# KogarashiNetwork/Kogarashi

Hardware: AMD Instinct MI355X
Metric: bn254_g1_msm_pairs_per_sec (higher is better)
Workload: dtype u32x9 (29-bit limbs)

## Files before the change

### kogarashi_amd/csrc/curve.h

```cpp
#pragma once
#include "fp29.h"
#include "fp_inv.h"

namespace kg {

template <class F>
struct Affine {
  F x, y;
};

template <class F>
struct XYZZ {
  F x, y, zz, zzz;
  static KG_HD XYZZ identity() { return {F::zero(), F::zero(), F::zero(), F::zero()}; }
};

template <class F>
KG_HD bool is_identity(const XYZZ<F>& p) { return is_zero_2p(p.zz); }

template <class F>
KG_HD XYZZ<F> from_affine(const Affine<F>& a) { return {a.x, a.y, F::one(), F::one()}; }

template <class F>
KG_HD XYZZ<F> double_affine(const Affine<F>& a) {
// ... 12 lines not shown
KG_HD XYZZ<F> double_xyzz(const XYZZ<F>& p) {
  if (is_identity(p)) return p;
  F u = norm(dbl(p.y));
  F v = sqr(u);
  F w = mul(u, v);
  F s = mul(p.x, v);
  F xx = sqr(p.x);
  F m = norm(add(dbl(xx), xx));
  F x3 = vred(norm(sub<4, 1>(sqr(m), norm(dbl(s)))));
  F y3 = vred(norm(sub<4, 1>(mul(m, norm(sub<4, 1>(s, x3))), mul(w, p.y))));
  return {x3, y3, mul(v, p.zz), mul(w, p.zzz)};
}

template <class F>
KG_HD XYZZ<F> add_mixed(const XYZZ<F>& p, const Affine<F>& a) {
  if (is_identity(p)) return from_affine(a);
  F u2 = mul(a.x, p.zz);
  F s2 = mul(a.y, p.zzz);
  F pp_ = norm(sub<4, 1>(u2, p.x));
  F r = norm(sub<4, 1>(s2, p.y));
  F pp = sqr(pp_);
  if (is_zero_2p(pp)) {
    if (is_zero(r)) return double_affine(a);
    return XYZZ<F>::identity();
  }
  F ppp = mul(pp_, pp);
  F q = mul(p.x, pp);
  F x3 = vred(norm(sub<8, 3>(sqr(r), add(ppp, dbl(q)))));
  F y3 = mul2sub(r, norm(sub<4, 1>(q, x3)), p.y, ppp);
  return {x3, y3, mul(p.zz, pp), mul(p.zzz, ppp)};
}

template <class F>
KG_HD XYZZ<F> add_mixed_signed(const XYZZ<F>& p, const Affine<F>& a, bool negate) {
  if (is_identity(p)) return from_affine(negate ? neg_affine(a) : a);
  F u2 = mul(a.x, p.zz);
  F s2 = mul(a.y, p.zzz);
  F pp_ = norm(sub<8, 1>(u2, p.x));
  F t = negate ? sub<8, 1>(F::zero(), s2) : s2;
  F r = norm(sub<4, 1>(t, p.y));
  F pp = sqr(pp_);
  if (is_zero_2p(pp)) {
    if (is_zero(r)) return double_affine(negate ? neg_affine(a) : a);
    return XYZZ<F>::identity();
  }
  F ppp = mul(pp_, pp);
  F q = mul(p.x, pp);
  F x3 = norm(sub<4, 3>(sqr(r), add(ppp, dbl(q))));
  F y3 = mul2sub(r, norm(sub<8, 1>(q, x3)), p.y, ppp);
  return {x3, y3, mul(p.zz, pp), mul(p.zzz, ppp)};
}

template <class G>
KG_HD XYZZ<Fp2<G>> add_mixed_signed(const XYZZ<Fp2<G>>& p, const Affine<Fp2<G>>& a, bool negate) {
  return add_mixed(p, negate ? neg_affine(a) : a);
}

template <class F>
KG_HD XYZZ<F> add_xyzz(const XYZZ<F>& p, const XYZZ<F>& q_) {
  if (is_identity(p)) return q_;
  if (is_identity(q_)) return p;
  F u1 = mul(p.x, q_.zz);
  F u2 = mul(q_.x, p.zz);
  F s1 = mul(p.y, q_.zzz);
  F s2 = mul(q_.y, p.zzz);
  F pp_ = norm(sub<4, 1>(u2, u1));
  F r = norm(sub<4, 1>(s2, s1));
  F pp = sqr(pp_);
  if (is_zero_2p(pp)) {
    if (is_zero(r)) return double_xyzz(p);
    return XYZZ<F>::identity();
  }
  F ppp = mul(pp_, pp);
  F q = mul(u1, pp);
  F x3 = vred(norm(sub<8, 3>(sqr(r), add(ppp, dbl(q)))));
  F y3 = mul2sub(r, norm(sub<4, 1>(q, x3)), s1, ppp);
  return {x3, y3, mul(mul(p.zz, q_.zz), pp), mul(mul(p.zzz, q_.zzz), ppp)};
}

#if defined(__HIP_DEVICE_COMPILE__)
#define KG_STREAM_FENCE() __asm__ volatile("" ::: "memory")
#else
#define KG_STREAM_FENCE() ((void)0)
#endif
// ... 83 lines not shown
```

### kogarashi_amd/csrc/fp29.h

```cpp
#pragma once
#include <type_traits>
#include <cstdint>
#include "fp_consts.h"

#if defined(__HIPCC__)
#include <hip/hip_runtime.h>
#define KG_HD __host__ __device__ __forceinline__
#else
#define KG_HD inline __attribute__((always_inline))
#endif

namespace kg {

constexpr uint32_t M29 = 0x1fffffffu;

template <class P>
struct Fp {
  using Params = P;
  uint32_t l[9];

  static KG_HD Fp zero() {
    Fp r;
#pragma unroll
    for (int i = 0; i < 9; ++i) r.l[i] = 0;
// ... 367 lines not shown
#pragma unroll
  for (int i = 0; i < 9; ++i) {
    z |= a.l[i];
    e |= a.l[i] ^ P::P[i];
  }
  return z == 0 || e == 0;
}
template <class P>
KG_HD bool is_zero(const Fp<P>& a) { return is_zero_2p(mul(a, Fp<P>::one())); }

template <class P>
KG_HD bool same_limbs(const Fp<P>& a, const Fp<P>& b) {
  uint32_t e = 0;
#pragma unroll
  for (int i = 0; i < 9; ++i) e |= a.l[i] ^ b.l[i];
  return e == 0;
}

template <class P>
KG_HD Fp<P> limbs_from_words(const uint32_t w[8]) {
  Fp<P> r;
  r.l[0] = w[0] & M29;
  r.l[1] = ((w[0] >> 29) | (w[1] << 3)) & M29;
  r.l[2] = ((w[1] >> 26) | (w[2] << 6)) & M29;
  r.l[3] = ((w[2] >> 23) | (w[3] << 9)) & M29;
  r.l[4] = ((w[3] >> 20) | (w[4] << 12)) & M29;
  r.l[5] = ((w[4] >> 17) | (w[5] << 15)) & M29;
  r.l[6] = ((w[5] >> 14) | (w[6] << 18)) & M29;
  r.l[7] = ((w[6] >> 11) | (w[7] << 21)) & M29;
  r.l[8] = w[7] >> 8;
  return r;
}
template <class P>
KG_HD void words_from_limbs(const Fp<P>& a, uint32_t w[8]) {
  w[0] = a.l[0] | (a.l[1] << 29);
  w[1] = (a.l[1] >> 3) | (a.l[2] << 26);
  w[2] = (a.l[2] >> 6) | (a.l[3] << 23);
  w[3] = (a.l[3] >> 9) | (a.l[4] << 20);
  w[4] = (a.l[4] >> 12) | (a.l[5] << 17);
  w[5] = (a.l[5] >> 15) | (a.l[6] << 14);
  w[6] = (a.l[6] >> 18) | (a.l[7] << 11);
  w[7] = (a.l[7] >> 21) | (a.l[8] << 8);
}
template <class P>
KG_HD Fp<P> from_ref(const uint32_t w[8]) { return mul(limbs_from_words<P>(w), Fp<P>::from_const(P::C_FROM_REF)); }
template <class P>
KG_HD void to_ref(const Fp<P>& a, uint32_t w[8]) {
  words_from_limbs(reduce_2p(mul(a, Fp<P>::from_const(P::C_TO_REF))), w);
}
template <class P>
KG_HD void ref_to_int(const uint32_t w[8], uint32_t k[8]) {
  words_from_limbs(reduce_2p(mul(limbs_from_words<P>(w), Fp<P>::from_const(P::C_REF_TO_INT))), k);
}
template <class P>
KG_HD Fp<P> from_int(const uint32_t w[8]) { return mul(limbs_from_words<P>(w), Fp<P>::from_const(P::C_INT_TO_MONT)); }
template <class P>
KG_HD void int_to_ref(const uint32_t k[8], uint32_t w[8]) {
  words_from_limbs(reduce_2p(mul(limbs_from_words<P>(k), Fp<P>::from_const(P::C_R2_REF))), w);
}

template <class P>
KG_HD Fp<P> pow_words(const Fp<P>& a, const uint32_t e[8]) {
  Fp<P> r = Fp<P>::one();
  for (int i = 255; i >= 0; --i) {
    r = sqr(r);
    if ((e[i >> 5] >> (i & 31)) & 1) r = mul(r, a);
  }
  return r;
}
template <class P>
KG_HD Fp<P> inv(const Fp<P>& a) {
  uint32_t e[8];
  Fp<P> pm2 = Fp<P>::from_const(P::P);
  pm2.l[0] -= 2;
  words_from_limbs(pm2, e);
  return pow_words(a, e);
}

template <class P>
// ... 87 lines not shown
```

### kogarashi_amd/csrc/fp29_checked.h

```cpp
#pragma once
#include <cstdio>
#include <cstdlib>
#include "fp29.h"

namespace kg {

struct BoundFail {
  static void fail(const char* what, double a, double b) {
    std::fprintf(stderr, "FpChecked: bound violated: %s (%.6g vs %.6g)\n", what, a, b);
    std::abort();
  }
};

template <class P>
struct FpChecked {
  using Params = P;
  Fp<P> v;
  double lb;
  double tb;
  double kb;

  static constexpr double RHO() { return 169.0; }
  static double ptop1() { return (double)P::PTOP + 1.0; }

// ... 130 lines not shown
  if (!(r.lb < 4294967296.0 && r.tb < 4294967296.0)) BoundFail::fail("sub limb overflow", r.lb, 4294967296.0);
  return r;
}
template <class P>
inline FpChecked<P> norm(const FpChecked<P>& a) {
  if (!(a.lb + a.lb / 536870912.0 + 1 < 4294967296.0)) BoundFail::fail("norm carry overflow", a.lb, 4294967296.0);
  double t = a.kb * FpChecked<P>::ptop1();
  double t2 = a.tb + a.lb / 536870912.0 + 1;
  FpChecked<P> r{norm(a.v), (double)M29, t < t2 ? t : t2, a.kb};
  r.check_actual();
  return r;
}
template <class P>
inline FpChecked<P> reduce_2p(const FpChecked<P>& a) {
  if (!(a.kb <= 2.0 + 1e-9 && a.lb <= (double)M29)) BoundFail::fail("reduce_2p input not in [0,2p) normalised", a.kb, 2.0);
  return {reduce_2p(a.v), (double)M29, FpChecked<P>::ptop1(), 1.0};
}
template <class P>
inline FpChecked<P> reduce(const FpChecked<P>& a) { return reduce_2p(mul(a, FpChecked<P>::one())); }
template <class P>
inline bool is_zero_2p(const FpChecked<P>& a) {
  if (!(a.kb <= 2.0 + 1e-9 && a.lb <= (double)M29)) BoundFail::fail("is_zero_2p input not in [0,2p) normalised", a.kb, 2.0);
  return is_zero_2p(a.v);
}
template <class P>
inline bool is_zero(const FpChecked<P>& a) { return is_zero_2p(mul(a, FpChecked<P>::one())); }
template <class P>
inline FpChecked<P> inv(const FpChecked<P>& a) {
  (void)mul(a, a);
  return {inv(a.v), (double)M29, 2.0 * FpChecked<P>::ptop1(), 2.0};
}

template <class P>
inline FpChecked<P> inv_fast(const FpChecked<P>& a) { return inv(a); }

using FqC = FpChecked<FqParams>;
using FrC = FpChecked<FrParams>;
using Fq2C = Fp2<FqC>;

}
```

### kogarashi_amd/csrc/msm_acc_kernels.h

```cpp
#pragma once
#include "msm_bases.h"
#include "msm_level_kernels.h"

namespace kg {
namespace msm {
namespace {

template <class F>
struct PointAoS {
  static constexpr int NW = PointIO<F>::NW;
  static __device__ __forceinline__ void store(uint32_t* base, size_t i, const XYZZ<F>& p) {
    uint32_t w[NW];
    pack(p, w);
    uint4* dst = reinterpret_cast<uint4*>(base + i * NW);
#pragma unroll
    for (int j = 0; j < NW / 4; ++j) dst[j] = make_uint4(w[4 * j], w[4 * j + 1], w[4 * j + 2], w[4 * j + 3]);
  }
  static __device__ __forceinline__ XYZZ<F> load(const uint32_t* base, size_t i) {
    uint32_t w[NW];
    const uint4* src = reinterpret_cast<const uint4*>(base + i * NW);
#pragma unroll
    for (int j = 0; j < NW / 4; ++j) { uint4 v = src[j]; w[4 * j] = v.x; w[4 * j + 1] = v.y; w[4 * j + 2] = v.z; w[4 * j + 3] = v.w; }
    return unpack(w);
  }
// ... 15 lines not shown
    constexpr int E = RawIO<F>::NW;
    XYZZ<F> p;
    get(p.x, w); get(p.y, w + E); get(p.zz, w + 2 * E); get(p.zzz, w + 3 * E);
    return p;
  }
};

template <class G>
struct PointAoS<Fp2S<G>> {
  using F = Fp2S<G>;
  static constexpr int NW = PointIO<F>::NW;
  static __device__ __forceinline__ void store(uint32_t* base, size_t i, const XYZZ<F>& p) {
    uint32_t w[36];
#pragma unroll
    for (int k = 0; k < 9; ++k) { w[k] = p.x.v.l[k]; w[9 + k] = p.y.v.l[k]; w[18 + k] = p.zz.v.l[k]; w[27 + k] = p.zzz.v.l[k]; }
    uint4* dst = reinterpret_cast<uint4*>(base + i * NW + 36 * F::half());
#pragma unroll
    for (int j = 0; j < 9; ++j) dst[j] = make_uint4(w[4 * j], w[4 * j + 1], w[4 * j + 2], w[4 * j + 3]);
  }
  static __device__ __forceinline__ XYZZ<F> load(const uint32_t* base, size_t i) {
    uint32_t w[36];
    const uint4* src = reinterpret_cast<const uint4*>(base + i * NW + 36 * F::half());
#pragma unroll
    for (int j = 0; j < 9; ++j) { uint4 v = src[j]; w[4 * j] = v.x; w[4 * j + 1] = v.y; w[4 * j + 2] = v.z; w[4 * j + 3] = v.w; }
    XYZZ<F> p;
#pragma unroll
    for (int k = 0; k < 9; ++k) { p.x.v.l[k] = w[k]; p.y.v.l[k] = w[9 + k]; p.zz.v.l[k] = w[18 + k]; p.zzz.v.l[k] = w[27 + k]; }
    return p;
  }
};


constexpr int MAX_FUSED = 3;
struct AccSets {
  int nsets;
  const uint32_t* pb[MAX_FUSED];
  uint32_t idx_off[MAX_FUSED];
  uint32_t* partial[MAX_FUSED];
  uint32_t tab_n[MAX_FUSED];
  uint8_t fmt64[MAX_FUSED];
};
template <class F> struct AccStore {
  static __device__ __forceinline__ void store(uint32_t* base, size_t i, const XYZZ<F>& p) { PointAoS<F>::store(base, i, p); }
};
template <class G> struct AccStore<Fp2S<G>> {
  static __device__ __forceinline__ void store(uint32_t* base, size_t i, const XYZZ<Fp2S<G>>& p) {
    uint32_t* dst = base + i * 72 + 9 * Fp2S<G>::half();
#pragma unroll
    for (int k = 0; k < 9; ++k) { dst[k] = p.x.v.l[k]; dst[18 + k] = p.y.v.l[k]; dst[36 + k] = p.zz.v.l[k]; dst[54 + k] = p.zzz.v.l[k]; }
  }
};
#ifdef KG_EXP_ACC_WAVES
template <class F> struct AccWaves { static constexpr int MIN = KG_EXP_ACC_WAVES; };
#else
template <class F> struct AccWaves { static constexpr int MIN = 1; };
#endif
template <class G> struct AccWaves<Fp2<G>> { static constexpr int MIN = 2; };
template <class F>
__global__ void __launch_bounds__(64) __attribute__((amdgpu_waves_per_eu(AccWaves<F>::MIN))) k_acc_tasks(AccSets A, const uint32_t* __restrict__ sorted,
                                                  const uint32_t* __restrict__ bstart, const uint32_t* __restrict__ bsize, Level L,
                                                  const uint32_t* __restrict__ task_bkt, const uint32_t* __restrict__ task_id,
                                                  size_t n, int W, int B, uint32_t T0, size_t pstride, int mshift, uint32_t T_top, int top_w) {
  const int set = A.nsets > 1 ? (int)(blockIdx.x % (unsigned)A.nsets) : 0;
  const uint32_t p = ((A.nsets > 1 ? blockIdx.x / (unsigned)A.nsets : blockIdx.x) * blockDim.x + threadIdx.x) / Lanes<F>::N;
  if (p >= L.base[W]) return;
  const uint32_t* __restrict__ pbases = A.pb[0];
  uint32_t idx_off = A.idx_off[0], tab_n = A.tab_n[0];
  bool fmt64 = A.fmt64[0] != 0;
  uint32_t* __restrict__ partial = A.partial[0];
#pragma unroll
  for (int k = 1; k < MAX_FUSED; ++k)
    if (set == k) { pbases = A.pb[k]; idx_off = A.idx_off[k]; partial = A.partial[k]; tab_n = A.tab_n[k]; fmt64 = A.fmt64[k] != 0; }
  const size_t bi = task_bkt[p];
  const uint32_t t = task_id[p];
  const int w = (int)(bi / B);
  const uint32_t seg = t - L.base[w] - L.rel[bi];
  const uint32_t len_all = bsize[bi];
  const uint32_t T = bucket_task_len(task_len(T0, T_top, w, top_w), len_all);
  const uint32_t lo = seg * T, hi = lo + T < len_all ? lo + T : len_all;
  const uint32_t* list = sorted + (size_t)w * n + bstart[bi];
  constexpr int PW = 2 * BaseIO<F>::PE;
  XYZZ<F> acc = XYZZ<F>::identity();
  for (uint32_t j = lo; j < hi; ++j) {
    const uint32_t e = list[j];
    uint32_t idx = e & 0x7fffffffu;
    size_t row = 0;
    if (mshift) { row = (size_t)(idx >> mshift) * tab_n; idx &= (1u << mshift) - 1u; }
    if (idx < idx_off) continue;
    Affine<F> a;
#ifdef KG_EXP_ACC_CACHED
    const size_t at = (row + (idx - idx_off)) & 0xffffu;
#else
    const size_t at = row + (idx - idx_off);
#endif
    if (fmt64 ? BaseIO<F>::load_point64(pbases + at * (2 * BaseIO<F>::PK), a.x, a.y) : BaseIO<F>::load_point(pbases + at * PW, a.x, a.y))
      continue;
    acc = add_mixed_signed(acc, a, (e & 0x80000000u) != 0);
  }
  AccStore<F>::store(partial, t, acc);
}

#ifdef KG_EXPERIMENTS
template <class F>
__global__ void __launch_bounds__(64) __attribute__((amdgpu_waves_per_eu(AccWaves<F>::MIN))) k_acc_tasks_q(AccSets A, const uint32_t* __restrict__ sorted,
                                                  const uint32_t* __restrict__ bstart, const uint32_t* __restrict__ bsize, Level L,
                                                  const uint32_t* __restrict__ task_bkt, const uint32_t* __restrict__ task_id,
                                                  size_t n, int W, int B, uint32_t T0, size_t pstride, int mshift, uint32_t T_top, int top_w) {
  __shared__ uint4 pf[4 * 64];
  typedef const __attribute__((address_space(1))) void* gptr_t;
  typedef __attribute__((address_space(3))) void* lptr_t;
  constexpr uint32_t NONE = 0xffffffffu;
  const int lane = threadIdx.x;
  const int set = A.nsets > 1 ? (int)(blockIdx.x % (unsigned)A.nsets) : 0;
  const uint32_t p = (A.nsets > 1 ? blockIdx.x / (unsigned)A.nsets : blockIdx.x) * blockDim.x + threadIdx.x;
  const bool live = p < L.base[W];
  const uint32_t* __restrict__ pbases = A.pb[0];
  uint32_t idx_off = A.idx_off[0], tab_n = A.tab_n[0];
  uint32_t* __restrict__ partial = A.partial[0];
#pragma unroll
  for (int k = 1; k < MAX_FUSED; ++k)
    if (set == k) { pbases = A.pb[k]; idx_off = A.idx_off[k]; partial = A.partial[k]; tab_n = A.tab_n[k]; }
  uint32_t t = 0, len = 0;
  const uint32_t* list = sorted;
  if (live) {
    const size_t bi = task_bkt[p];
    t = task_id[p];
    const int w = (int)(bi / B);
    const uint32_t seg = t - L.base[w] - L.rel[bi];
    const uint32_t len_all = bsize[bi];
    const uint32_t T = bucket_task_len(task_len(T0, T_top, w, top_w), len_all);
// ... 20 lines not shown
        __builtin_amdgcn_global_load_lds((gptr_t)src, (lptr_t)(pf + k * 64), 16, 0, 0);
      }
    }
  };
  XYZZ<F> acc = XYZZ<F>::identity();
  uint32_t e1 = len > 0 ? list[0] : NONE, e2 = len > 1 ? list[1] : NONE;
  request(e1);
  const int slot = 64 * (lane >> 4) + 4 * (lane & 15);
  for (uint32_t j = 0; j < mx; ++j) {
    uint32_t wd[16];
#pragma unroll
    for (int k = 0; k < 4; ++k) { const uint4 v = pf[slot + k]; wd[4 * k] = v.x; wd[4 * k + 1] = v.y; wd[4 * k + 2] = v.z; wd[4 * k + 3] = v.w; }
    const uint32_t e = e1;
    asm volatile("s_waitcnt lgkmcnt(0)" ::: "memory");
    e1 = e2;
    request(e1);
    e2 = j + 2 < len ? list[j + 2] : NONE;
    if (locate(e) == NONE) continue;
    Affine<F> a;
    if (BaseIO<F>::point64_from_words(wd, a.x, a.y)) continue;
    acc = add_mixed_signed(acc, a, (e & 0x80000000u) != 0);
  }
  if (live) AccStore<F>::store(partial, t, acc);
}

template <class F> struct PfField { using T = Fq; static constexpr bool ok = false; };
template <class P> struct PfField<Fp<P>> { using T = Fp<P>; static constexpr bool ok = true; };
template <class F>
static int acc_prefetch(const AccSets& A, int njobs, size_t nbases) {
  if (!PfField<F>::ok) return 0;
  const int mode = tuning().acc_prefetch, from_log = tuning().acc_prefetch_log;
  if (mode == 0 || nbases < ((size_t)1 << from_log)) return 0;
  for (int k = 0; k < njobs; ++k)
    if (!A.fmt64[k]) return 0;
  return mode;
}
#endif

template <class F>
__global__ void __launch_bounds__(256) k_gather_buckets(const uint32_t* __restrict__ pin, size_t in_stride, Level L, int W, int B,
                                                        uint32_t* __restrict__ buckets) {
  KG_REDUCE_PRIO();
  const size_t t = ((size_t)blockIdx.x * blockDim.x + threadIdx.x) / Lanes<F>::N;
  const size_t total = (size_t)W * B;
  if (t >= total) return;
  const int w = (int)(t / B);
  XYZZ<F> p = XYZZ<F>::identity();
  if (L.cnt[t]) p = PointAoS<F>::load(pin, (size_t)L.base[w] + L.rel[t]);
  PointIO<F>::store(buckets, total, t, p);
}

template <class F, class KF> struct PartialIO {
  static __device__ __forceinline__ XYZZ<KF> load(const uint32_t* base, size_t i) { return PointAoS<F>::load(base, i); }
};
template <class G> struct PartialIO<Fp2<G>, Fp2S<G>> {
  static __device__ __forceinline__ XYZZ<Fp2S<G>> load(const uint32_t* base, size_t i) {
    const uint32_t* src = base + i * 72 + 9 * Fp2S<G>::half();
    XYZZ<Fp2S<G>> p;
#pragma unroll
    for (int k = 0; k < 9; ++k) { p.x.v.l[k] = src[k]; p.y.v.l[k] = src[18 + k]; p.zz.v.l[k] = src[36 + k]; p.zzz.v.l[k] = src[54 + k]; }
    return p;
  }
};

}
}
}
// ... 1 lines not shown
```

### kogarashi_amd/csrc/msm_bases.h

```cpp
#pragma once
#include "msm_common.h"

namespace kg {
namespace msm {
namespace {

template <class F> struct FieldOf;
template <class Q> struct FieldOf<Fp<Q>> { using P = Q; };
template <class G> struct FieldOf<Fp2<G>> { using P = typename G::Params; };
template <class F> struct BaseIO;
template <class P> struct BaseIO<Fp<P>> {
  static constexpr int W = 8;
  static constexpr int PE = 9;
  static __device__ __forceinline__ void convert(const uint64_t* src, uint32_t* dst) {
    uint32_t w[8];
    load_words(src, 0, w);
    const Fp<P> v = from_ref<P>(w);
#pragma unroll
    for (int j = 0; j < 9; ++j) dst[j] = v.l[j];
  }
  static __device__ __forceinline__ Fp<P> from_words(const uint32_t* w) {
    Fp<P> r;
#pragma unroll
    for (int j = 0; j < 9; ++j) r.l[j] = w[j];
    return r;
  }
  static constexpr int PK = 8;
  static __device__ __forceinline__ void pack(const Fp<P>& v, uint32_t* dst) { words_from_limbs(v, dst); }
  static __device__ __forceinline__ bool load_point64(const uint32_t* src, Fp<P>& x, Fp<P>& y) {
    uint32_t w[16];
    const uint4* p = reinterpret_cast<const uint4*>(src);
#pragma unroll
    for (int j = 0; j < 4; ++j) { const uint4 v = p[j]; w[4 * j] = v.x; w[4 * j + 1] = v.y; w[4 * j + 2] = v.z; w[4 * j + 3] = v.w; }
    const bool inf = (w[7] & INF_BIT) != 0;
    w[7] &= ~INF_BIT;
    x = limbs_from_words<P>(w); y = limbs_from_words<P>(w + 8);
    return inf;
  }
  static __device__ __forceinline__ bool point64_from_words(uint32_t (&w)[16], Fp<P>& x, Fp<P>& y) {
    const bool inf = (w[7] & INF_BIT) != 0;
    w[7] &= ~INF_BIT;
    x = limbs_from_words<P>(w); y = limbs_from_words<P>(w + 8);
    return inf;
  }
  static __device__ __forceinline__ bool load_point(const uint32_t* src, Fp<P>& x, Fp<P>& y) {
    uint32_t w[18];
    const uint2* p = reinterpret_cast<const uint2*>(src);
#pragma unroll
    for (int j = 0; j < 9; ++j) { const uint2 v = p[j]; w[2 * j] = v.x; w[2 * j + 1] = v.y; }
    const bool inf = (w[8] & INF_BIT) != 0;
    w[8] &= ~INF_BIT;
    x = from_words(w); y = from_words(w + 9);
    return inf;
  }
};
template <class F> struct BaseIO<Fp2<F>> {
  static constexpr int W = 16;
  static constexpr int PE = 18;
  static __device__ __forceinline__ void convert(const uint64_t* src, uint32_t* dst) {
    BaseIO<F>::convert(src, dst);
    BaseIO<F>::convert(src + 4, dst + 9);
  }
  static constexpr int PK = 16;
  static __device__ __forceinline__ void pack(const Fp2<F>& v, uint32_t* dst) { BaseIO<F>::pack(v.c0, dst); BaseIO<F>::pack(v.c1, dst + 8); }
  static __device__ __forceinline__ bool load_point64(const uint32_t* src, Fp2<F>& x, Fp2<F>& y) {
    uint32_t w[32];
    const uint4* p = reinterpret_cast<const uint4*>(src);
#pragma unroll
    for (int j = 0; j < 8; ++j) { const uint4 v = p[j]; w[4 * j] = v.x; w[4 * j + 1] = v.y; w[4 * j + 2] = v.z; w[4 * j + 3] = v.w; }
    const bool inf = (w[7] & INF_BIT) != 0;
    w[7] &= ~INF_BIT;
    using P = typename F::Params;
    x = {limbs_from_words<P>(w), limbs_from_words<P>(w + 8)};
    y = {limbs_from_words<P>(w + 16), limbs_from_words<P>(w + 24)};
    return inf;
  }
  static __device__ __forceinline__ bool load_point(const uint32_t* src, Fp2<F>& x, Fp2<F>& y) {
    uint32_t w[36];
    const uint4* p = reinterpret_cast<const uint4*>(src);
#pragma unroll
    for (int j = 0; j < 9; ++j) { const uint4 v = p[j]; w[4 * j] = v.x; w[4 * j + 1] = v.y; w[4 * j + 2] = v.z; w[4 * j + 3] = v.w; }
    const bool inf = (w[8] & INF_BIT) != 0;
    w[8] &= ~INF_BIT;
    x = {BaseIO<F>::from_words(w), BaseIO<F>::from_words(w + 9)};
    y = {BaseIO<F>::from_words(w + 18), BaseIO<F>::from_words(w + 27)};
    return inf;
  }
};


}
}
template <class F> struct RawIO<Fp2S<F>> {
  static constexpr int NW = 18;
  static __device__ __forceinline__ Fp2S<F> load(const uint32_t* base, size_t stride, size_t i) {
    return {RawIO<F>::load(base + (size_t)(9 * Fp2S<F>::half()) * stride, stride, i)};
  }
  static __device__ __forceinline__ void store(uint32_t* base, size_t stride, size_t i, const Fp2S<F>& a) {
    RawIO<F>::store(base + (size_t)(9 * Fp2S<F>::half()) * stride, stride, i, a.v);
  }
};
namespace msm {
namespace {

template <class G> struct BaseIO<Fp2S<G>> {
  static constexpr int W = 16, PE = 18, PK = 16;
  using P = typename G::Params;
  static __device__ __forceinline__ bool load_point64(const uint32_t* src, Fp2S<G>& x, Fp2S<G>& y) {
    const int h = Fp2S<G>::half();
    const uint4* p = reinterpret_cast<const uint4*>(src);
    uint32_t w[16];
    const uint4 a0 = p[2 * h], a1 = p[2 * h + 1], b0 = p[4 + 2 * h], b1 = p[5 + 2 * h];
    w[0] = a0.x; w[1] = a0.y; w[2] = a0.z; w[3] = a0.w; w[4] = a1.x; w[5] = a1.y; w[6] = a1.z; w[7] = a1.w;
    w[8] = b0.x; w[9] = b0.y; w[10] = b0.z; w[11] = b0.w; w[12] = b1.x; w[13] = b1.y; w[14] = b1.z; w[15] = b1.w;
    int flag = (h == 0 && (w[7] & INF_BIT) != 0) ? 1 : 0;
    flag |= __shfl_xor(flag, 1);
    if (h == 0) w[7] &= ~INF_BIT;
    x.v = limbs_from_words<P>(w); y.v = limbs_from_words<P>(w + 8);
    return flag != 0;
  }
  static __device__ __forceinline__ bool load_point(const uint32_t* src, Fp2S<G>& x, Fp2S<G>& y) {
    const int h = Fp2S<G>::half();
    uint32_t wx[9], wy[9];
#pragma unroll
    for (int k = 0; k < 9; ++k) { wx[k] = src[9 * h + k]; wy[k] = src[18 + 9 * h + k]; }
    int flag = (h == 0 && (wx[8] & INF_BIT) != 0) ? 1 : 0;
    flag |= __shfl_xor(flag, 1);
    if (h == 0) wx[8] &= ~INF_BIT;
    x.v = BaseIO<G>::from_words(wx); y.v = BaseIO<G>::from_words(wy);
    return flag != 0;
  }
};

template <class F>
__device__ __forceinline__ void store_resident(uint32_t* out, size_t i, uint32_t* buf , int fmt64) {
  constexpr int PE = BaseIO<F>::PE, PK = BaseIO<F>::PK;
  if (fmt64) {
    const bool inf = (buf[8] & INF_BIT) != 0;
    buf[8] &= ~INF_BIT;
// ... 71 lines not shown
```

### kogarashi_amd/csrc/msm_host.cpp

```cpp
#include "common.h"
#include "host_fp.h"
#include "msm_internal.h"
#include <algorithm>
#include <chrono>
#include <cstdlib>
#include <cstring>
#include <condition_variable>
#include <mutex>
#include <thread>

using namespace kg;

namespace {

struct G1Cfg { using HF = HostFq; static constexpr int E64 = 4; static constexpr int ID = KG_G1; };
struct GkCfg { using HF = HostFr; static constexpr int E64 = 4; static constexpr int ID = KG_GRUMPKIN; };
struct G2Cfg { using HF = HostFq2; static constexpr int E64 = 8; static constexpr int ID = KG_G2; };

template <class HF> struct HostIO;
template <class P> struct HostIO<HostFp<P>> {
  static HostFp<P> load(const uint64_t* w) { return HostFp<P>::from_words(w); }
  static void store(const HostFp<P>& a, uint64_t* w) { a.to_words(w); }
};
template <class F> struct HostIO<Fp2<F>> {
// ... 148 lines not shown
    rc = kg::msm_sort(ctx, sfield, d_scalars + 4 * a, cnt, &S, j > 0);
    if (rc != KG_OK) break;
    rc = kg::msm_run(ctx, S, curve, d_bases + a * pw, d_inf ? d_inf + a : nullptr, cnt, 0, 16 + j);
    if (rc != KG_OK) break;
    uint64_t* out = part[j];
    fin[j] = kg::pool(ctx).submit([ctx, curve, j, out] { return kg::msm_finish(ctx, curve, 16 + j, out); });
  }
  ctx->msm_window = saved_window;
  for (int j = 0; j < K; ++j)
    if (fin[j].valid()) { const int r2 = fin[j].get(); if (rc == KG_OK) rc = r2; }
  if (rc != KG_OK) { kg_ctx_sync(ctx); return rc; }
  return sum_slices(ctx, curve, part, K, out_xyz);
}

static int msm_grouped(kg_ctx* ctx, int curve, const uint64_t* d_bases, const uint8_t* d_inf, const uint64_t* d_scalars, size_t n, const int* gw, int NG,
                       uint64_t* out_xyz) {
  KG_HIP(ctx, hipSetDevice(ctx->device));
  if (!ctx->side_stream) KG_TRY(make_side_stream(ctx));
  KG_TRY(make_sort_stream(ctx));
  for (int g = 1; g < NG && g < ctx->tune.group_accq; ++g)
    if (!ctx->acc_stream[g]) KG_HIP(ctx, create_stream(ctx, &ctx->acc_stream[g].h, false));
  kg::MsmSortPlan Q;
  const int main_first = ctx->tune.group_main_first;
  KG_TRY(kg::msm_sort_begin(ctx, curve == KG_GRUMPKIN ? KG_FQ : KG_FR, d_scalars, n, &Q, false, 0, 1, NG, gw, main_first != 0));
  if (main_first == 1) {
    KG_HIP(ctx, hipEventRecord(ctx->ev_prep, ctx->stream));
    KG_HIP(ctx, hipStreamWaitEvent(ctx->sort_stream, ctx->ev_prep, 0));
  }
  bool resident = false;
  size_t off = 0;
  for (const auto& r : ctx->registered)
    if (covers(r, curve, d_bases, d_inf, n, &off)) { resident = true; break; }
  const bool f64 = resident_fmt64(n);
  if (!resident) {
    const size_t bytes = n * (f64 ? (curve == KG_G2 ? 128 : 64) : (curve == KG_G2 ? 144 : 72));
    KG_TRY(ctx->ws_pb.ensure(DevMem{ctx, "resident-bases allocation"}, bytes, bytes / 8));
    hipStream_t cq = ctx->side_stream;
    if (!ctx->inputs_complete) {
      KG_HIP(ctx, hipEventRecord(ctx->ev_order, ctx->stream));
      KG_HIP(ctx, hipStreamWaitEvent(cq, ctx->ev_order, 0));
    }
    PhaseScope ph(ctx, "prep_bases", cq);
    prep_bases_enqueue(curve, cq, d_bases, d_inf, n, ctx->ws_pb.as<uint32_t>(), f64);
    ph.end();
    KG_HIP(ctx, hipGetLastError());
    KG_HIP(ctx, hipEventRecord(ctx->ev_pb, cq));
  }
  kg::MsmSorted S[kg_ctx::MAX_GROUPS];
  int slots[kg_ctx::MAX_GROUPS];
  int rc = kg::msm_sort_group(ctx, Q, 0, &S[0], main_first != 0);
  if (rc == KG_OK && main_first == 2) KG_HIP(ctx, hipStreamWaitEvent(ctx->sort_stream, S[0].ready, 0));
  if (rc == KG_OK && NG > 1) rc = kg::msm_sort_group(ctx, Q, 1, &S[1]);
  int launched = 0;
  for (int g = 0; g < NG && rc == KG_OK; ++g) {
    rc = kg::msm_sort_wait(ctx, &S[g]);
    if (rc != KG_OK) break;
    const int accq = ctx->tune.group_accq;
    S[g].acc_stream = (accq > 1 && g % accq) ? ctx->acc_stream[g % accq] : nullptr;
    const int rinl = ctx->tune.group_reduce_inline;
    S[g].reduce_inline = rinl && g == NG - 1;
    S[g].tail_alone = g == NG - 1;
    const int one_side = ctx->tune.group_one_side;
    slots[g] = one_side ? 16 + 2 * g : 16 + g;
    kg::MsmRunJob job{d_bases, d_inf, n, 0u, slots[g], false, resident ? nullptr : ctx->ws_pb.as<const uint32_t>(), f64};
    rc = kg::msm_run_multi(ctx, S[g], curve, &job, 1);
    if (rc != KG_OK) break;
// ... 358 lines not shown
```

### kogarashi_amd/csrc/msm_internal.h

```cpp
#pragma once
#include "common.h"

namespace kg {

int pick_window(size_t n, int forced);
bool resident_fmt64(size_t n);
bool table_fmt64();
void prep_bases_enqueue(int curve, hipStream_t st, const uint64_t* d_bases, const uint8_t* d_inf, size_t n, uint32_t* out, bool fmt64);
void table_next_enqueue(int curve, hipStream_t st, const uint32_t* prev, size_t n, int c, uint32_t* next, bool fmt64);
void host_trace(const char* what);

}
```

### kogarashi_amd/csrc/msm_run.hip

```cpp
#include "msm_reduce_kernels.h"
#include <cstdlib>
#include <cstring>

using namespace kg;
using namespace kg::msm;

namespace kg {
void prep_bases_enqueue(int curve, hipStream_t st, const uint64_t* d_bases, const uint8_t* d_inf, size_t n, uint32_t* out, bool fmt64) {
  if (curve == KG_G1) launch_prep_bases<Fq>(st, d_bases, d_inf, n, out, fmt64);
  else if (curve == KG_GRUMPKIN) launch_prep_bases<Fr>(st, d_bases, d_inf, n, out, fmt64);
  else launch_prep_bases<Fq2>(st, d_bases, d_inf, n, out, fmt64);
}
void table_next_enqueue(int curve, hipStream_t st, const uint32_t* prev, size_t n, int c, uint32_t* next, bool fmt64) {
  const dim3 grid((unsigned)((n + 63) / 64));
  if (curve == KG_G1) hipLaunchKernelGGL(k_table_next<Fq>, grid, dim3(64), 0, st, prev, n, c, next, fmt64 ? 1 : 0);
  else if (curve == KG_GRUMPKIN) hipLaunchKernelGGL(k_table_next<Fr>, grid, dim3(64), 0, st, prev, n, c, next, fmt64 ? 1 : 0);
  else hipLaunchKernelGGL(k_table_next<Fq2>, grid, dim3(64), 0, st, prev, n, c, next, fmt64 ? 1 : 0);
}
}

namespace kg {

template <class Cfg>
int msm_run_multi_t(kg_ctx* ctx, const MsmSorted& S, const MsmRunJob* jobs, int njobs) {
  using F = typename Cfg::F;
  using KF = typename Cfg::KF;
  constexpr unsigned LPT = Lanes<KF>::N;
  constexpr int PW = 2 * BaseIO<F>::PE;
  constexpr int NW = PointIO<F>::NW;
  if (njobs < 1 || njobs > MAX_FUSED) return set_err(ctx, KG_ERR_BAD_ARG, "bad number of fused base arrays");
  const int W = S.W, B = S.B, c = S.c;
  const size_t npts = S.npts, part_cap = S.part_cap, nexp = (size_t)W * c;
  const size_t exp_bytes = nexp * 4 * Cfg::E64 * 8;
  hipStream_t st = S.acc_stream ? S.acc_stream : ctx->stream, sq;
  KG_TRY(scalar_queue(ctx, &sq));
  bool ordered_bases = false, converted = false, shared_pb = false;
  if (!ctx->side_stream) KG_TRY(make_side_stream(ctx));
  if (st != ctx->stream && !ctx->inputs_complete) {
    KG_HIP(ctx, hipEventRecord(ctx->ev_order, ctx->stream));
    KG_HIP(ctx, hipStreamWaitEvent(st, ctx->ev_order, 0));
  }
  struct Lay { size_t o_pb, o_lc[2], o_lr[2], o_lb[2], o_part[2], o_pbuf[2], o_rowtot, o_misc, o_hot; char* ws; const uint32_t* pb; int set; };
  Lay lay[MAX_FUSED];
  AccSets A;
  A.nsets = njobs;
  for (int k = 0; k < MAX_FUSED; ++k) { A.pb[k] = nullptr; A.idx_off[k] = 0; A.partial[k] = nullptr; A.tab_n[k] = 0; A.fmt64[k] = 0; }
  for (int k = 0; k < njobs; ++k) {
    const MsmRunJob& J = jobs[k];
    Lay& Y = lay[k];
    Carver cv;
    const uint32_t* reg_pb = nullptr;
    if (J.packed) {
      if (S.merged_shift) return set_err(ctx, KG_ERR_BAD_ARG, "merged sort against caller-converted bases");
      reg_pb = J.packed; A.fmt64[k] = J.packed64 ? 1 : 0; shared_pb = true;
    }
    for (const auto& r : ctx->registered) {
      if (reg_pb) break;
      size_t off = 0;
      if (!covers(r, Cfg::ID, J.d_bases, J.d_inf, J.nbases, &off)) continue;
      if (S.merged_shift) {
        if (!r.table || r.table_c != c || r.table_W != S.windows) continue;
        reg_pb = r.table.as<uint32_t>() + off * (r.table64 ? 2 * BaseIO<F>::PK : PW);
        A.tab_n[k] = (uint32_t)r.n;
        A.fmt64[k] = r.table64 ? 1 : 0;
      } else {
        reg_pb = r.packed.as<uint32_t>() + off * (r.fmt64 ? 2 * BaseIO<F>::PK : PW);
        A.fmt64[k] = r.fmt64 ? 1 : 0;
      }
      break;
    }
    if (S.merged_shift && !reg_pb) return set_err(ctx, KG_ERR_BAD_ARG, "merged sort against bases without a matching window table");
    const bool conv64 = !reg_pb && resident_fmt64(J.nbases);
    if (conv64) A.fmt64[k] = 1;
    Y.o_pb = cv.take(reg_pb ? 256 : J.nbases * (conv64 ? 2 * BaseIO<F>::PK : PW) * 4);
    for (int i = 0; i < 2; ++i) {
      Y.o_lc[i] = cv.take(npts * 4); Y.o_lr[i] = cv.take(npts * 4); Y.o_lb[i] = cv.take((size_t)(W + 1) * 4);
      Y.o_part[i] = cv.take(part_cap * NW * 4); Y.o_pbuf[i] = cv.take(npts * NW * 4);
    }
    Y.o_rowtot = cv.take((size_t)W * 4); Y.o_misc = cv.take(64);
    Y.o_hot = cv.take(S.nhot ? (size_t)(S.nhot < HOT_MAX ? S.nhot : HOT_MAX) * hot_split<KF>(S.max_cnt) * NW * 4 : 0);
    Y.set = J.slot % kg_ctx::RUN_SETS;
    for (int k2 = 0; k2 < k; ++k2)
      if (lay[k2].set == Y.set) return set_err(ctx, KG_ERR_BAD_ARG, "fused MSMs need result slots in different run-space sets");
    KG_TRY(ctx->ws_run[Y.set].ensure(DevMem{ctx, "msm run-space allocation"}, cv.off, cv.off / 8));
    KG_TRY(ensure_slot(ctx, J.slot, exp_bytes));
    KG_HIP(ctx, create_events({ctx->ev_acc[Y.set]}));
    Y.ws = (char*)ctx->ws_run[Y.set].get();
    Y.pb = reg_pb ? reg_pb : (uint32_t*)(Y.ws + Y.o_pb);
    for (int s2 = 0; s2 < kg_ctx::NSLOTS; ++s2)
      if (s2 % kg_ctx::RUN_SETS == Y.set && ctx->slots[s2].done && ctx->slots[s2].busy) {
        KG_HIP(ctx, hipStreamWaitEvent(st, ctx->slots[s2].done, 0));
        if (!reg_pb) KG_HIP(ctx, hipStreamWaitEvent(sq, ctx->slots[s2].done, 0));
        ctx->slots[s2].busy = false;
      }
    if (!reg_pb) {
      if (!ctx->inputs_complete && !ordered_bases && !J.bases_complete) {
        KG_HIP(ctx, hipEventRecord(ctx->ev_order, st));
        KG_HIP(ctx, hipStreamWaitEvent(sq, ctx->ev_order, 0));
        ordered_bases = true;
      }
      PhaseScope ph(ctx, "prep_bases", sq);
      launch_prep_bases<F>(sq, J.d_bases, J.d_inf, J.nbases, (uint32_t*)(Y.ws + Y.o_pb), conv64);
      ph.end();
      converted = true;
    }
    A.pb[k] = Y.pb; A.idx_off[k] = J.idx_off; A.partial[k] = (uint32_t*)(Y.ws + Y.o_part[0]);
// ... 181 lines not shown
```

### kogarashi_amd/csrc/tuning.h

```cpp
#pragma once
#include <string>

#define KG_TUNING_TABLE(X)                                                                                                                   \
   \
  X(wide_window, "KG_WIDE_WINDOW", 23, "log2 of the length from which a blocking MSM takes the 20-bit window (13 windows, unsliced, window groups); 0 = never (index slices with c = 17)") \
  X(msm_groups, "KG_MSM_GROUPS", -1, "window groups of a blocking MSM: -1 automatic, 0/1 none, k = k equal groups; a list \"a,b,c\" names the groups' window counts from the top window down") \
  X(msm_sliced, "KG_MSM_SLICED", 1, "0 = a blocking MSM of 2^23 pairs or more runs in window groups instead of four index slices") \
  X(msm_t, "KG_MSM_T", -1, "task length of the accumulation (entries per lane): -1 = 2 n / B + 16") \
  X(merged_t, "KG_MERGED_T", -1, "task length of a merged (window-table) accumulation: -1 = one resident round of lanes") \
  X(hot_shift, "KG_HOT_SHIFT", -1, "hot buckets are cut 2^shift times finer: -1 = 2 (0 for a merged sort)") \
  X(hot_sum, "KG_HOT_SUM", 1, "0 = hot buckets go through the generic partial-sum rounds instead of the workgroup-wide trees") \
  X(gather_fuse, "KG_GATHER_FUSE", 1, "0 = the bucket gather writes the dense bucket array instead of fusing the first halving level") \
  X(fmt64_min_log, "KG_FMT64_MIN_LOG", 0, "log2 of the array length from which resident bases take the 64-byte point form (30 = always the 72-byte limb form)") \
  X(table64, "KG_TABLE64", 1, "0 = window tables in the 72-byte limb form") \
  X(pipe_accq, "KG_PIPE_ACCQ", 1, "2 = MSM tickets alternate between two accumulation queues (measured level; off)") \
  X(coop_tail, "KG_COOP_TAIL", 1, "0 = the last reduction of a blocking MSM runs the streamed tail kernel (96 VGPRs) instead of the lane-cooperative one") \
  X(small_max, "KG_SMALL_MAX", 32768, "longest MSM (pairs) that runs as the short-input kernel (msm_small.hip): 0 = never, at most 32768 (G2: 20480)") \
  X(small_max_flight, "KG_SMALL_MAX_FLIGHT", 8192, "longest MSM begun with kg_msm_begin that runs as the short-input kernel (a call in flight shares the chip with its neighbours, and the kernel's grid fills it at these lengths); G2: half of it") \
  X(small_glv, "KG_SMALL_GLV", 1, "short-input MSMs of up to 16384 pairs split every scalar into two 127-bit halves k1 + k2 lambda against P and (beta x, y): half the windows, half the host chain (0 = off, 1 = where it pays: G1 / Grumpkin up to 6144 pairs, G2 up to 16384, 2 = wherever the index field allows)") \
  X(small_kt_from, "KG_SMALL_KT_FROM", 2048, "short-input MSMs LONGER than this convert their scalars once, by a launch of their own, instead of in every workgroup (0 = always)") \
  X(small_c, "KG_SMALL_C", 0, "window width of the short-input kernel: 0 = by length, 2..10") \
  X(small_r, "KG_SMALL_R", -1, "log2 of the buckets a workgroup of the short-input kernel owns: -1 = by length, 0..7 (2^(c-1-r) workgroups per window)") \
   \
  X(sort_nch, "KG_SORT_NCH", 64, "cap on the scalar chunks (workgroups per window) of the first sort pass, 1..1024") \
  X(sort_alone, "KG_SORT_ALONE", 1, "0 = every sort is shaped for a busy device (a blocking call's first sort normally takes the whole chip)") \
  X(gs_tile, "KG_GS_TILE", -1, "entries per tile of the first sort pass: -1 = 4096 (8192 for the wide windows), 0 = the 1024-entry kernel (needs -DKG_EXPERIMENTS)") \
  X(gs_nt, "KG_GS_NT", 0, "threads per workgroup of the first sort pass beside an accumulation: 0 = 256 (512 for the wide windows)") \
  X(gs_nt0, "KG_GS_NT0", 1024, "threads per workgroup of the first sort pass on an idle device") \
   \
  X(group_main_first, "KG_GROUP_MAIN_FIRST", 0, "1 / 2 = conversion and first group's sort on the main queue (measured slower; off)") \
  X(group_accq, "KG_GROUP_ACCQ", 2, "accumulation queues the window groups rotate over") \
  X(group_reduce_inline, "KG_GROUP_REDUCE_INLINE", 1, "the last group's bucket reduction follows its accumulation on the same queue") \
  X(blocking_reduce_inline, "KG_BLOCKING_REDUCE_INLINE", 1, "an unsplit blocking MSM (8193 .. 2^17 pairs, window tables) runs its bucket reduction behind the accumulation on the main queue instead of handing it to a reduction queue") \
  X(group_one_side, "KG_GROUP_ONE_SIDE", 0, "1 = all groups reduce on one side queue") \
   \
  X(host_slices, "KG_HOST_SLICES", 0, "index slices a host-scalar MSM is uploaded and run in: 0 = automatic (by length), 1..8") \
  X(host_first_div, "KG_HOST_FIRST_DIV", 0, "the first slice (whose upload nothing hides) is 1/div of an equal share: 0 = automatic") \
  X(blocking_tables_log, "KG_BLOCKING_TABLES_LOG", 18, "longest blocking kg_msm (log2 pairs) that goes through the window tables of registered bases; longer ones run in window groups") \
  X(host_slice_tables, "KG_HOST_SLICE_TABLES", 1, "index slices of a host-scalar MSM go through the window tables of registered bases when they have them") \
  X(host_accq, "KG_HOST_ACCQ", 2, "accumulation queues the slices of a host-scalar MSM alternate over (1 = the main queue only)") \
   \
  X(small_stamps, "KG_SMALL_STAMPS", 0, "experiment: 1 = the short-input kernel stamps its phase boundaries; the previous call's phase times go to stderr (tools/dbg/small_stamps.py)") \
  X(acc_prefetch, "KG_ACC_PREFETCH", 0, "experiment: 1 = accumulation with the next base prefetched into LDS (k_acc_tasks_q; measured level)") \
  X(acc_prefetch_log, "KG_ACC_PREFETCH_LOG", 0, "experiment: log2 of the array length from which KG_ACC_PREFETCH applies") \
  X(g2_pair_acc, "KG_G2_PAIR_ACC", 0, "experiment: 1 = G2 accumulation on lane pairs (~150 VGPRs instead of 250; measured level)") \
   \
  X(g16_h_early, "KG_G16_H_EARLY", 1, "order of h's transform chain in a proof: 1 = before the fused G1 accumulation, 0 = last (the order up to round 3), 2 = in front of the G2 accumulation") \
// ... 30 lines not shown
```

Measured before the change: 781.0 million.

## Gather caller-held G1 bases directly in accumulation instead of converting per call

Unregistered G1/Grumpkin base arrays without identity flags, when 16-byte aligned, are now read in their caller (Montgomery x32 ABI) form directly by the accumulation kernel rather than first being converted to the resident 64-byte form each call. The point loader unpacks the 32-bit words into 29-bit limbs of 32·value, and the mixed add runs on those scaled coordinates, converting with a divide-by-32 and a Montgomery multiply only in the rare identity or doubling branches. This removes a conversion pass and its scratch allocation per MSM, in exchange for a slightly heavier gather inside the hot loop and an extra format branch.

```diff
diff --git a/kogarashi_amd/csrc/curve.h b/kogarashi_amd/csrc/curve.h
--- a/kogarashi_amd/csrc/curve.h
+++ b/kogarashi_amd/csrc/curve.h
@@ -68,8 +68,14 @@
 }
 
 template <class F>
-KG_HD XYZZ<F> add_mixed_signed(const XYZZ<F>& p, const Affine<F>& a, bool negate) {
-  if (is_identity(p)) return from_affine(negate ? neg_affine(a) : a);
+KG_HD Affine<F> affine_from_abi(const Affine<F>& a) { return {from_ref_x32(a.x), from_ref_x32(a.y)}; }
+
+template <class F>
+KG_HD XYZZ<F> add_mixed_signed(const XYZZ<F>& p, const Affine<F>& a, bool negate, bool abi) {
+  if (is_identity(p)) {
+    const Affine<F> b = abi ? affine_from_abi(a) : a;
+    return from_affine(negate ? neg_affine(b) : b);
+  }
   F u2 = mul(a.x, p.zz);
   F s2 = mul(a.y, p.zzz);
   F pp_ = norm(sub<8, 1>(u2, p.x));
@@ -77,7 +83,10 @@
   F r = norm(sub<4, 1>(t, p.y));
   F pp = sqr(pp_);
   if (is_zero_2p(pp)) {
-    if (is_zero(r)) return double_affine(negate ? neg_affine(a) : a);
+    if (is_zero(r)) {
+      const Affine<F> b = abi ? affine_from_abi(a) : a;
+      return double_affine(negate ? neg_affine(b) : b);
+    }
     return XYZZ<F>::identity();
   }
   F ppp = mul(pp_, pp);
@@ -86,6 +95,8 @@
   F y3 = mul2sub(r, norm(sub<8, 1>(q, x3)), p.y, ppp);
   return {x3, y3, mul(p.zz, pp), mul(p.zzz, ppp)};
 }
+template <class F>
+KG_HD XYZZ<F> add_mixed_signed(const XYZZ<F>& p, const Affine<F>& a, bool negate) { return add_mixed_signed(p, a, negate, false); }
 
 template <class G>
 KG_HD XYZZ<Fp2<G>> add_mixed_signed(const XYZZ<Fp2<G>>& p, const Affine<Fp2<G>>& a, bool negate) {
diff --git a/kogarashi_amd/csrc/fp29.h b/kogarashi_amd/csrc/fp29.h
--- a/kogarashi_amd/csrc/fp29.h
+++ b/kogarashi_amd/csrc/fp29.h
@@ -423,6 +423,28 @@
   return r;
 }
 template <class P>
+KG_HD Fp<P> limbs_from_words_x32(const uint32_t w[8]) {
+  Fp<P> r;
+  r.l[0] = (w[0] << 5) & M29;
+  r.l[1] = ((w[0] >> 24) | (w[1] << 8)) & M29;
+  r.l[2] = ((w[1] >> 21) | (w[2] << 11)) & M29;
+  r.l[3] = ((w[2] >> 18) | (w[3] << 14)) & M29;
+  r.l[4] = ((w[3] >> 15) | (w[4] << 17)) & M29;
+  r.l[5] = ((w[4] >> 12) | (w[5] << 20)) & M29;
+  r.l[6] = ((w[5] >> 9) | (w[6] << 23)) & M29;
+  r.l[7] = ((w[6] >> 6) | (w[7] << 26)) & M29;
+  r.l[8] = w[7] >> 3;
+  return r;
+}
+template <class P>
+KG_HD Fp<P> limbs_div32(const Fp<P>& a) {
+  Fp<P> r;
+#pragma unroll
+  for (int i = 0; i < 8; ++i) r.l[i] = (a.l[i] >> 5) | ((a.l[i + 1] & 31u) << 24);
+  r.l[8] = a.l[8] >> 5;
+  return r;
+}
+template <class P>
 KG_HD void words_from_limbs(const Fp<P>& a, uint32_t w[8]) {
   w[0] = a.l[0] | (a.l[1] << 29);
   w[1] = (a.l[1] >> 3) | (a.l[2] << 26);
@@ -436,6 +458,8 @@
 template <class P>
 KG_HD Fp<P> from_ref(const uint32_t w[8]) { return mul(limbs_from_words<P>(w), Fp<P>::from_const(P::C_FROM_REF)); }
 template <class P>
+KG_HD Fp<P> from_ref_x32(const Fp<P>& a) { return mul(limbs_div32(a), Fp<P>::from_const(P::C_FROM_REF)); }
+template <class P>
 KG_HD void to_ref(const Fp<P>& a, uint32_t w[8]) {
   words_from_limbs(reduce_2p(mul(a, Fp<P>::from_const(P::C_TO_REF))), w);
 }
diff --git a/kogarashi_amd/csrc/fp29_checked.h b/kogarashi_amd/csrc/fp29_checked.h
--- a/kogarashi_amd/csrc/fp29_checked.h
+++ b/kogarashi_amd/csrc/fp29_checked.h
@@ -186,6 +186,22 @@
 }
 
 template <class P>
+inline FpChecked<P> checked_from_words_x32(const uint32_t w[8]) {
+  FpChecked<P> r{limbs_from_words_x32<P>(w), (double)M29, 32.0 * FpChecked<P>::ptop1(), 32.0};
+  r.check_actual();
+  return r;
+}
+template <class P>
+inline FpChecked<P> from_ref_x32(const FpChecked<P>& a) {
+  a.check_actual();
+  if (!(a.lb <= (double)M29)) BoundFail::fail("from_ref_x32 input limbs not normalised", a.lb, (double)M29);
+  if (a.v.l[0] & 31u) BoundFail::fail("from_ref_x32 input is not 32 x a value", a.v.l[0] & 31u, 0);
+  const FpChecked<P> v{limbs_div32(a.v), (double)M29, a.tb / 32.0, a.kb / 32.0};
+  v.check_actual();
+  return mul(v, FpChecked<P>::from_const(P::C_FROM_REF));
+}
+
+template <class P>
 inline FpChecked<P> inv_fast(const FpChecked<P>& a) { return inv(a); }
 
 using FqC = FpChecked<FqParams>;
diff --git a/kogarashi_amd/csrc/msm_acc_kernels.h b/kogarashi_amd/csrc/msm_acc_kernels.h
--- a/kogarashi_amd/csrc/msm_acc_kernels.h
+++ b/kogarashi_amd/csrc/msm_acc_kernels.h
@@ -71,13 +71,18 @@
 
 
 constexpr int MAX_FUSED = 3;
+enum : uint8_t {
+  BASES_72 = 0,
+  BASES_64 = 1,
+  BASES_ABI = 2
+};
 struct AccSets {
   int nsets;
   const uint32_t* pb[MAX_FUSED];
   uint32_t idx_off[MAX_FUSED];
   uint32_t* partial[MAX_FUSED];
   uint32_t tab_n[MAX_FUSED];
-  uint8_t fmt64[MAX_FUSED];
+  uint8_t fmt[MAX_FUSED];
 };
 template <class F> struct AccStore {
   static __device__ __forceinline__ void store(uint32_t* base, size_t i, const XYZZ<F>& p) { PointAoS<F>::store(base, i, p); }
@@ -105,11 +110,11 @@
   if (p >= L.base[W]) return;
   const uint32_t* __restrict__ pbases = A.pb[0];
   uint32_t idx_off = A.idx_off[0], tab_n = A.tab_n[0];
-  bool fmt64 = A.fmt64[0] != 0;
+  uint32_t fmt = A.fmt[0];
   uint32_t* __restrict__ partial = A.partial[0];
 #pragma unroll
   for (int k = 1; k < MAX_FUSED; ++k)
-    if (set == k) { pbases = A.pb[k]; idx_off = A.idx_off[k]; partial = A.partial[k]; tab_n = A.tab_n[k]; fmt64 = A.fmt64[k] != 0; }
+    if (set == k) { pbases = A.pb[k]; idx_off = A.idx_off[k]; partial = A.partial[k]; tab_n = A.tab_n[k]; fmt = A.fmt[k]; }
   const size_t bi = task_bkt[p];
   const uint32_t t = task_id[p];
   const int w = (int)(bi / B);
@@ -132,9 +137,18 @@
 #else
     const size_t at = row + (idx - idx_off);
 #endif
-    if (fmt64 ? BaseIO<F>::load_point64(pbases + at * (2 * BaseIO<F>::PK), a.x, a.y) : BaseIO<F>::load_point(pbases + at * PW, a.x, a.y))
-      continue;
-    acc = add_mixed_signed(acc, a, (e & 0x80000000u) != 0);
+    if constexpr (BaseIO<F>::HAS_ABI) {
+      const bool abi = fmt == BASES_ABI;
+      bool inf = false;
+      if (abi) BaseIO<F>::load_point_abi(pbases + at * 16, a.x, a.y);
+      else inf = fmt == BASES_64 ? BaseIO<F>::load_point64(pbases + at * (2 * BaseIO<F>::PK), a.x, a.y) : BaseIO<F>::load_point(pbases + at * PW, a.x, a.y);
+      if (inf) continue;
+      acc = add_mixed_signed(acc, a, (e & 0x80000000u) != 0, abi);
+    } else {
+      if (fmt == BASES_64 ? BaseIO<F>::load_point64(pbases + at * (2 * BaseIO<F>::PK), a.x, a.y) : BaseIO<F>::load_point(pbases + at * PW, a.x, a.y))
+        continue;
+      acc = add_mixed_signed(acc, a, (e & 0x80000000u) != 0);
+    }
   }
   AccStore<F>::store(partial, t, acc);
 }
@@ -221,7 +235,7 @@
   const int mode = tuning().acc_prefetch, from_log = tuning().acc_prefetch_log;
   if (mode == 0 || nbases < ((size_t)1 << from_log)) return 0;
   for (int k = 0; k < njobs; ++k)
-    if (!A.fmt64[k]) return 0;
+    if (A.fmt[k] != BASES_64) return 0;
   return mode;
 }
 #endif
diff --git a/kogarashi_amd/csrc/msm_bases.h b/kogarashi_amd/csrc/msm_bases.h
--- a/kogarashi_amd/csrc/msm_bases.h
+++ b/kogarashi_amd/csrc/msm_bases.h
@@ -37,6 +37,14 @@
     x = limbs_from_words<P>(w); y = limbs_from_words<P>(w + 8);
     return inf;
   }
+  static constexpr bool HAS_ABI = true;
+  static __device__ __forceinline__ void load_point_abi(const uint32_t* src, Fp<P>& x, Fp<P>& y) {
+    uint32_t w[16];
+    const uint4* p = reinterpret_cast<const uint4*>(src);
+#pragma unroll
+    for (int j = 0; j < 4; ++j) { const uint4 v = p[j]; w[4 * j] = v.x; w[4 * j + 1] = v.y; w[4 * j + 2] = v.z; w[4 * j + 3] = v.w; }
+    x = limbs_from_words_x32<P>(w); y = limbs_from_words_x32<P>(w + 8);
+  }
   static __device__ __forceinline__ bool point64_from_words(uint32_t (&w)[16], Fp<P>& x, Fp<P>& y) {
     const bool inf = (w[7] & INF_BIT) != 0;
     w[7] &= ~INF_BIT;
@@ -57,6 +65,7 @@
 template <class F> struct BaseIO<Fp2<F>> {
   static constexpr int W = 16;
   static constexpr int PE = 18;
+  static constexpr bool HAS_ABI = false;
   static __device__ __forceinline__ void convert(const uint64_t* src, uint32_t* dst) {
     BaseIO<F>::convert(src, dst);
     BaseIO<F>::convert(src + 4, dst + 9);
@@ -105,6 +114,7 @@
 
 template <class G> struct BaseIO<Fp2S<G>> {
   static constexpr int W = 16, PE = 18, PK = 16;
+  static constexpr bool HAS_ABI = false;
   using P = typename G::Params;
   static __device__ __forceinline__ bool load_point64(const uint32_t* src, Fp2S<G>& x, Fp2S<G>& y) {
     const int h = Fp2S<G>::half();
diff --git a/kogarashi_amd/csrc/msm_host.cpp b/kogarashi_amd/csrc/msm_host.cpp
--- a/kogarashi_amd/csrc/msm_host.cpp
+++ b/kogarashi_amd/csrc/msm_host.cpp
@@ -204,6 +204,7 @@
   for (const auto& r : ctx->registered)
     if (covers(r, curve, d_bases, d_inf, n, &off)) { resident = true; break; }
   const bool f64 = resident_fmt64(n);
+  if (!resident && kg::acc_abi_bases(ctx, curve, d_bases, d_inf, n)) resident = true;
   if (!resident) {
     const size_t bytes = n * (f64 ? (curve == KG_G2 ? 128 : 64) : (curve == KG_G2 ? 144 : 72));
     KG_TRY(ctx->ws_pb.ensure(DevMem{ctx, "resident-bases allocation"}, bytes, bytes / 8));
diff --git a/kogarashi_amd/csrc/msm_internal.h b/kogarashi_amd/csrc/msm_internal.h
--- a/kogarashi_amd/csrc/msm_internal.h
+++ b/kogarashi_amd/csrc/msm_internal.h
@@ -6,6 +6,7 @@
 int pick_window(size_t n, int forced);
 bool resident_fmt64(size_t n);
 bool table_fmt64();
+bool acc_abi_bases(const kg_ctx* ctx, int curve, const uint64_t* d_bases, const uint8_t* d_inf, size_t n);
 void prep_bases_enqueue(int curve, hipStream_t st, const uint64_t* d_bases, const uint8_t* d_inf, size_t n, uint32_t* out, bool fmt64);
 void table_next_enqueue(int curve, hipStream_t st, const uint32_t* prev, size_t n, int c, uint32_t* next, bool fmt64);
 void host_trace(const char* what);
diff --git a/kogarashi_amd/csrc/msm_run.hip b/kogarashi_amd/csrc/msm_run.hip
--- a/kogarashi_amd/csrc/msm_run.hip
+++ b/kogarashi_amd/csrc/msm_run.hip
@@ -10,6 +10,9 @@
   if (curve == KG_G1) launch_prep_bases<Fq>(st, d_bases, d_inf, n, out, fmt64);
   else if (curve == KG_GRUMPKIN) launch_prep_bases<Fr>(st, d_bases, d_inf, n, out, fmt64);
   else launch_prep_bases<Fq2>(st, d_bases, d_inf, n, out, fmt64);
+}
+bool acc_abi_bases(const kg_ctx* ctx, int curve, const uint64_t* d_bases, const uint8_t* d_inf, size_t n) {
+  return ctx->tune.acc_abi_bases != 0 && (curve == KG_G1 || curve == KG_GRUMPKIN) && !d_inf && resident_fmt64(n) && ((uintptr_t)d_bases & 15) == 0;
 }
 void table_next_enqueue(int curve, hipStream_t st, const uint32_t* prev, size_t n, int c, uint32_t* next, bool fmt64) {
   const dim3 grid((unsigned)((n + 63) / 64));
@@ -44,7 +47,7 @@
   Lay lay[MAX_FUSED];
   AccSets A;
   A.nsets = njobs;
-  for (int k = 0; k < MAX_FUSED; ++k) { A.pb[k] = nullptr; A.idx_off[k] = 0; A.partial[k] = nullptr; A.tab_n[k] = 0; A.fmt64[k] = 0; }
+  for (int k = 0; k < MAX_FUSED; ++k) { A.pb[k] = nullptr; A.idx_off[k] = 0; A.partial[k] = nullptr; A.tab_n[k] = 0; A.fmt[k] = BASES_72; }
   for (int k = 0; k < njobs; ++k) {
     const MsmRunJob& J = jobs[k];
     Lay& Y = lay[k];
@@ -52,7 +55,7 @@
     const uint32_t* reg_pb = nullptr;
     if (J.packed) {
       if (S.merged_shift) return set_err(ctx, KG_ERR_BAD_ARG, "merged sort against caller-converted bases");
-      reg_pb = J.packed; A.fmt64[k] = J.packed64 ? 1 : 0; shared_pb = true;
+      reg_pb = J.packed; A.fmt[k] = J.packed64 ? BASES_64 : BASES_72; shared_pb = true;
     }
     for (const auto& r : ctx->registered) {
       if (reg_pb) break;
@@ -62,16 +65,20 @@
         if (!r.table || r.table_c != c || r.table_W != S.windows) continue;
         reg_pb = r.table.as<uint32_t>() + off * (r.table64 ? 2 * BaseIO<F>::PK : PW);
         A.tab_n[k] = (uint32_t)r.n;
-        A.fmt64[k] = r.table64 ? 1 : 0;
+        A.fmt[k] = r.table64 ? BASES_64 : BASES_72;
       } else {
         reg_pb = r.packed.as<uint32_t>() + off * (r.fmt64 ? 2 * BaseIO<F>::PK : PW);
-        A.fmt64[k] = r.fmt64 ? 1 : 0;
+        A.fmt[k] = r.fmt64 ? BASES_64 : BASES_72;
       }
       break;
     }
     if (S.merged_shift && !reg_pb) return set_err(ctx, KG_ERR_BAD_ARG, "merged sort against bases without a matching window table");
+    if (!reg_pb && BaseIO<F>::HAS_ABI && acc_abi_bases(ctx, Cfg::ID, J.d_bases, J.d_inf, J.nbases)) {
+      reg_pb = reinterpret_cast<const uint32_t*>(J.d_bases);
+      A.fmt[k] = BASES_ABI;
+    }
     const bool conv64 = !reg_pb && resident_fmt64(J.nbases);
-    if (conv64) A.fmt64[k] = 1;
+    if (conv64) A.fmt[k] = BASES_64;
     Y.o_pb = cv.take(reg_pb ? 256 : J.nbases * (conv64 ? 2 * BaseIO<F>::PK : PW) * 4);
     for (int i = 0; i < 2; ++i) {
       Y.o_lc[i] = cv.take(npts * 4); Y.o_lr[i] = cv.take(npts * 4); Y.o_lb[i] = cv.take((size_t)(W + 1) * 4);
diff --git a/kogarashi_amd/csrc/tuning.h b/kogarashi_amd/csrc/tuning.h
--- a/kogarashi_amd/csrc/tuning.h
+++ b/kogarashi_amd/csrc/tuning.h
@@ -13,6 +13,7 @@
   X(gather_fuse, "KG_GATHER_FUSE", 1, "0 = the bucket gather writes the dense bucket array instead of fusing the first halving level") \
   X(fmt64_min_log, "KG_FMT64_MIN_LOG", 0, "log2 of the array length from which resident bases take the 64-byte point form (30 = always the 72-byte limb form)") \
   X(table64, "KG_TABLE64", 1, "0 = window tables in the 72-byte limb form") \
+  X(acc_abi_bases, "KG_ACC_ABI_BASES", 1, "0 = an unregistered G1 / Grumpkin array without identity flags is converted to the resident form on every call instead of being gathered by the accumulation as the caller holds it") \
   X(pipe_accq, "KG_PIPE_ACCQ", 1, "2 = MSM tickets alternate between two accumulation queues (measured level; off)") \
   X(coop_tail, "KG_COOP_TAIL", 1, "0 = the last reduction of a blocking MSM runs the streamed tail kernel (96 VGPRs) instead of the lane-cooperative one") \
   X(small_max, "KG_SMALL_MAX", 32768, "longest MSM (pairs) that runs as the short-input kernel (msm_small.hip): 0 = never, at most 32768 (G2: 20480)") \
```

New measurement: 799.5 million (median of 6 runs). 1.02x the previous value.
